# zz9tf/FIA-KDD-19

Hardware: AMD Instinct MI355X
Metric: influence queries/sec (whole node) + % HBM roofline, MF k=16 ML-1M-ex (higher is better)
Workload: dtype f64

## Files before the change

### fia-kdd-19_amd/csrc/common.h

```cpp
#pragma once

#include <hip/hip_runtime.h>
#include <hip/hip_ext.h>
#include <cstdint>
#include <cstdio>
#include <string>
#include <vector>

#include "fia.h"

namespace fia {

constexpr int kWave = 64;
constexpr int kScoreThreads = 256;
constexpr int kScoreRows = 4;
constexpr int kChunk = 64 * kScoreRows;
constexpr int kRunQB = 16;
constexpr int kRunChunk = 128;
constexpr int kNcfRunChunk = 64;
constexpr int kRunUserCost = 3;

struct ChunkDesc {
  int64_t list_base;
  int64_t out_base;
  int32_t q;
  int32_t pos0;
  int32_t len;
  int32_t side;
};
constexpr int kPrepThreads = 256;
constexpr int kSolveThreads = 64;
constexpr int kGramChunk = 256;
constexpr int kGsSub = 16;
constexpr int kGsSlice = 256;
constexpr int kGsTarget = 8;
constexpr uint32_t kGsNoRow = 0x7fffff00u;
constexpr int kGsRing = 8;
constexpr int kGsMaxSub = 48;
constexpr int kGsMaxSeg = 4;
constexpr int kMfmaQB = 16;
constexpr int kMfmaCPI = 4;
constexpr int kWgBlocks = 4;
constexpr int kQueryBlock = 8;
static_assert(kGsSlice < 512, "a Gram-stream segment's count rides in 9 bits of its descriptor (out >> 23)");

struct DevBuf {
  void* ptr = nullptr;
  size_t bytes = 0;
  hipError_t reserve(size_t want, hipStream_t s) {
    if (want <= bytes && ptr) return hipSuccess;
    hipStreamCaptureStatus cs = hipStreamCaptureStatusNone;
    if (hipStreamIsCapturing(s, &cs) == hipSuccess && cs != hipStreamCaptureStatusNone)
      return hipErrorStreamCaptureUnsupported;
    size_t cap = want < 256 ? 256 : want;
    if (ptr) {
      const size_t grown = bytes + bytes / 4;
      if (grown > cap) cap = grown;
      hipError_t e = hipFreeAsync(ptr, s);
      if (e != hipSuccess) return e;
      ptr = nullptr;
      bytes = 0;
    }
    hipError_t e = hipMallocAsync(&ptr, cap, s);
    if (e == hipSuccess) bytes = cap; else ptr = nullptr;
    return e;
  }
  void release(hipStream_t s) {
    if (ptr) (void)hipFreeAsync(ptr, s);
    ptr = nullptr;
    bytes = 0;
  }
  template <class T> T* as() const { return reinterpret_cast<T*>(ptr); }
};

struct Side {
  DevBuf ptr;
  DevBuf row;
  DevBuf other;
  DevBuf rating;
};

struct Index {
  int64_t N = 0, U = 0, I = 0;
  Side side[2];
  DevBuf order[2];
  DevBuf gitems[2], gcomb[2];
  int64_t n_gitems[2] = {0, 0}, n_gcomb[2] = {0, 0}, n_gslots[2] = {0, 0};
  DevBuf pkey;
  DevBuf pcnt;
  DevBuf psum;
  int64_t pcap = 0;
  std::vector<int64_t> hptr[2];
  std::vector<int32_t> hord[2];
  int64_t gchunk = 0;
  DevBuf gsdesc, gsids, gswave, gscomb[2];
  int64_t n_gsw = 0, n_gsdesc = 0, n_gscomb[2] = {0, 0}, n_gsslots[2] = {0, 0};
  uint64_t gs_version = ~0ull;
  int gs_k = 0;
  uint64_t version = 0;
  bool valid = false;
};

#define FIA_SMALL_SIZES(X) X(MF, 8) X(MF, 16) X(MF, 32) X(MF, 64) X(NCF, 8) X(NCF, 16) X(NCF, 32)
#define FIA_BIG_SIZES(X) X(MF, 128) X(MF, 256) X(NCF, 64) X(NCF, 128) X(NCF, 256)

#define FIA_SIZE_CASE(fam, kv)                \
  if (model == FIA_MODEL_##fam && k == kv) {  \
    f(fam<kv>{});                             \
    return true;                              \
  }
template <template <int> class MF, template <int> class NCF, class F>
bool for_small_size(int model, int k, F&& f) {
  FIA_SMALL_SIZES(FIA_SIZE_CASE)
  return false;
}
template <template <int> class MF, template <int> class NCF, class F>
bool for_big_size(int model, int k, F&& f) {
  FIA_BIG_SIZES(FIA_SIZE_CASE)
  return false;
}
#undef FIA_SIZE_CASE

template <class I, class T>
__device__ __forceinline__ I last_at_most(const T* __restrict__ off, I lo, I hi, T g) {
  while (lo < hi) {
    const I mid = (lo + hi + 1) >> 1;
    if (off[mid] <= g) lo = mid; else hi = mid - 1;
  }
  return lo;
}

constexpr unsigned long long kEmptyKey = ~0ull;

__host__ __device__ inline unsigned long long pair_hash(unsigned long long k) {
  k += 0x9e3779b97f4a7c15ull;
  k = (k ^ (k >> 30)) * 0xbf58476d1ce4e5b9ull;
  k = (k ^ (k >> 27)) * 0x94d049bb133111ebull;
  return k ^ (k >> 31);
}

struct PairTable {
  const unsigned long long* key;
  const int32_t* cnt;
  const double* sum;
  unsigned long long mask;
  __device__ inline void lookup(unsigned long long k, double& c, double& s) const {
    unsigned long long h = pair_hash(k) & mask;
    c = 0.0;
    s = 0.0;
    for (unsigned long long probe = 0; probe <= mask; ++probe) {
      unsigned long long kk = key[h];
      if (kk == k) { c = (double)cnt[h]; s = sum[h]; return; }
      if (kk == kEmptyKey) return;
      h = (h + 1) & mask;
    }
  }
  __device__ inline void probe_start(unsigned long long k, unsigned long long& h, unsigned long long& kk) const {
    h = pair_hash(k) & mask;
    kk = key[h];
  }
  __device__ inline void probe_finish(unsigned long long k, unsigned long long h, unsigned long long kk, double& c,
                                      double& s) const {
    c = 0.0;
    s = 0.0;
    for (unsigned long long probe = 0; probe <= mask; ++probe) {
      if (kk == k) { c = (double)cnt[h]; s = sum[h]; return; }
      if (kk == kEmptyKey) return;
      h = (h + 1) & mask;
      kk = key[h];
    }
  }
};

struct Params {
  int model = -1, k = 0;
  int64_t U = 0, I = 0;
  const float* t[10] = {};
  double wd = 0.0, damping = 0.0;
  bool valid = false;
};

struct PhaseEvents {
  std::vector<std::pair<hipEvent_t, hipEvent_t>> ev[FIA_NUM_PHASES];
  std::vector<hipEvent_t> pool;
};

struct RecHead {
  static constexpr int inv_n = 0;
  static constexpr int c_q = 1;
  static constexpr int x_v = 2;
  static constexpr int rhat = 3;
};

}

struct fia_ctx {
  int device = 0;
  std::string err;
  fia::Params p;
  fia::Index idx;
  fia::DevBuf gram[2];
  fia::DevBuf l1[2];
  fia::DevBuf gpart[2];
  bool prepared = false;
  fia::DevBuf rec;
  fia::DevBuf coff;
  fia::DevBuf cdesc;
  fia::DevBuf cand_pos;
  fia::DevBuf cand_val;
  fia::DevBuf qscan;
  fia::DevBuf flag;
  fia::DevBuf nch;
  fia::DevBuf coupled;
  fia::DevBuf gcnt;
  fia::DevBuf gstart;
  fia::DevBuf grank;
  fia::DevBuf gq;
  fia::DevBuf qbase;
  fia::DevBuf slices;
  fia::DevBuf wstart;
  fia::DevBuf gscan;
  fia::DevBuf witems;
  fia::DevBuf d1tab;
  fia::DevBuf tkeys, tvals, tagg, tslot, tword, tsort;
  fia::DevBuf rowrec, gxq;
  uint64_t rowrec_version = ~0ull;
  fia::DevBuf dwork, dslab, dpairs;
  fia::DevBuf self[2];
  uint64_t self_version = ~0ull;
  fia::DevBuf resid;
  fia::DevBuf gm[2];
  fia::DevBuf wfrag;
  fia::DevBuf slot[2];
  fia::DevBuf mark;
  bool subset = false;
  bool small_subset = false;
  fia::DevBuf bitems[2], bcomb[2];
  int64_t n_bitems[2] = {0, 0}, n_bcomb[2] = {0, 0}, n_bslots[2] = {0, 0}, n_bcache[2] = {0, 0};
  uint64_t bitems_version = ~0ull;
  int bitems_k = 0;
  fia::DevBuf qwork;
  fia::DevBuf xb;
  fia::DevBuf syslist;
  fia::DevBuf cpllist;
  fia::DevBuf lscr;
  int num_cus = 0;
  hipStream_t stream = nullptr;
  bool has_stream = false;
  hipStream_t aux = nullptr;
  hipEvent_t fork_ev = nullptr, prep_ev = nullptr;
  bool prep_pending = false;
  hipEvent_t l1_ev = nullptr;
  bool l1_pending = false;
  unsigned profiling = 0;
  fia::PhaseEvents events;
};

namespace fia {

struct ModelArgs {
  int64_t U, I;
  const int64_t* ptr[2];
  const float* t[10];
  const double* l1[2];
  double wd;
};
template <class Args>
void fill_model_args(const fia_ctx* c, Args& A) {
  A.U = c->p.U;
  A.I = c->p.I;
  for (int s = 0; s < 2; ++s) {
    A.ptr[s] = c->idx.side[s].ptr.as<int64_t>();
    A.l1[s] = c->l1[s].as<double>();
  }
  for (int j = 0; j < 10; ++j) A.t[j] = c->p.t[j];
  A.wd = c->p.wd;
}

inline PairTable pair_table(const Index& X) {
  return {X.pkey.as<unsigned long long>(), X.pcnt.as<int32_t>(), X.psum.as<double>(),
          (unsigned long long)(X.pcap - 1)};
}

template <class Args>
void fill_list_args(const fia_ctx* c, Args& A) {
  fill_model_args(c, A);
  for (int s = 0; s < 2; ++s) {
    A.row[s] = c->idx.side[s].row.as<int32_t>();
    A.other[s] = c->idx.side[s].other.as<int32_t>();
    A.rating[s] = c->idx.side[s].rating.as<float>();
    A.gram[s] = c->gram[s].as<double>();
  }
  A.damping = c->p.damping;
  A.pairs = pair_table(c->idx);
}

hipError_t build_index(fia_ctx* c, int64_t N, int64_t U, int64_t I, const int32_t* user,
                       const int32_t* item, const float* rating, hipStream_t s, std::string& why);
hipError_t count_related(fia_ctx* c, int64_t Q, const int32_t* qu, const int32_t* qi,
                         int64_t* offsets, hipStream_t s);
hipError_t write_related(fia_ctx* c, int64_t Q, const int32_t* qu, const int32_t* qi,
                         const int64_t* offsets, int32_t* rel, hipStream_t s);
hipError_t build_chunks(fia_ctx* c, int64_t Q, const int32_t* qu, const int32_t* qi, const int64_t* offsets,
                        int64_t max_chunks, bool offsets_only, hipStream_t s, int32_t* zero_word = nullptr,
                        bool runs = false, int slice_cost = 0, int run_chunk = kRunChunk);
hipError_t build_gram_lists(fia_ctx* c, int64_t chunk, hipStream_t s);
hipError_t build_gram_stream(fia_ctx* c, int k, hipStream_t s);
hipError_t build_groups(fia_ctx* c, int64_t Q, const int32_t* qu, const int32_t* qi, const int64_t* offsets,
                        int64_t max_items, int qb, hipStream_t s, int cpi = 1);

hipError_t prepare_model(fia_ctx* c, hipStream_t s, bool& unsupported);
hipStream_t prepare_stream(fia_ctx* c, hipStream_t s);
hipError_t prepare_record(fia_ctx* c, hipStream_t ps, hipStream_t s);
hipError_t join_prepare(fia_ctx* c, hipStream_t s);
hipError_t join_l1(fia_ctx* c, hipStream_t s);
hipError_t prepare_model_for(fia_ctx* c, int64_t Q, const int32_t* qu, const int32_t* qi, hipStream_t s, hipStream_t ps,
                             bool& unsupported, bool mark_only);
hipError_t mark_entities(fia_ctx* c, int64_t Q, const int32_t* qu, const int32_t* qi, hipStream_t s);
hipError_t check_cover_small(fia_ctx* c, int64_t Q, const int32_t* qu, const int32_t* qi, int32_t* flag,
                             hipStream_t s);
hipError_t query_model(fia_ctx* c, int64_t Q, const int32_t* qu, const int32_t* qi, const int64_t* offsets,
                       int64_t max_chunks, int32_t* rel_idx, double* influence, double* x_out, int K,
                       int64_t* topk_pos, int64_t* topk_idx, double* topk_val, hipStream_t s,
                       bool& unsupported,
                       const double* x_in = nullptr);
int model_num_params(int model, int k);
bool model_supported(int model, int k);

bool big_supported(int model, int k);
hipError_t ensure_self(fia_ctx* c, hipStream_t s);
int live_contexts(int device);
hipError_t prepare_big(fia_ctx* c, int64_t Q, const int32_t* qu, const int32_t* qi, hipStream_t s);
hipError_t check_cover(fia_ctx* c, int64_t Q, const int32_t* qu, const int32_t* qi, int32_t* flag, hipStream_t s);
hipError_t query_big(fia_ctx* c, int64_t Q, const int32_t* qu, const int32_t* qi, const int64_t* offsets,
                     int64_t max_chunks, int32_t* rel_idx, double* influence, double* x_out, int K,
                     int64_t* topk_pos, int64_t* topk_idx, double* topk_val, hipStream_t s,
                     const double* x_in = nullptr);
struct PhaseSpan {
  hipEvent_t a = nullptr, b = nullptr;
};
struct QueryArgs;
struct GramStreamArgs {
  const int2* desc;
  const uint32_t* ids;
  const int32_t* wave;
  int64_t n_waves;
  const float* emb_other[2];
  uint32_t bytes_other[2];
  double* gram[2];
  double* part[2];
  const uint8_t* mark;
  int64_t moff[2];
};
hipError_t launch_gram_mf_stream(int k, const GramStreamArgs& G, hipStream_t s);
hipError_t launch_score_mf_runs(int k, int64_t grid, hipStream_t s, const QueryArgs& A, int64_t Q,
                                const ChunkDesc* cdesc, const int64_t* qbase, const int32_t* slices,
                                const double* rec, int32_t* rel_idx, double* influence, int K, int32_t* cand_pos,
                                double* cand_val, PhaseSpan ps);
hipError_t launch_score_ncf_runs(int k, int64_t grid, hipStream_t s, const QueryArgs& A, int64_t Q,
                                 const ChunkDesc* cdesc, const int64_t* qbase, const int32_t* slices,
                                 const double* rec, int32_t* rel_idx, double* influence, int K, int32_t* cand_pos,
                                 double* cand_val, PhaseSpan ps);
hipError_t launch_score_mf_mfma(int k, bool full, int64_t grid, hipStream_t s, PhaseSpan ps, const QueryArgs& A,
                                int64_t nE, const int64_t* wstart, const int32_t* witems, const int64_t* gstart,
                                const int32_t* gq, const int64_t* qbase, const double* rec, int32_t* rel_idx,
                                double* influence, int K, int32_t* cand_pos, double* cand_val);
hipError_t launch_topk_merge(fia_ctx* c, int64_t Q, const int32_t* qu, const int32_t* qi, int K, int spc,
                             int64_t* topk_pos, int64_t* topk_idx, double* topk_val, hipStream_t s,
                             int64_t max_chunks);

hipError_t score_candidates(fia_ctx* c, int64_t Q, const int32_t* qu, const int32_t* qi, const double* x,
                            const int64_t* cand_offsets, int64_t total_cand, const int32_t* cand_user,
                            const int32_t* cand_item, const float* cand_rating, double* influence, int K,
                            int64_t* topk_pos, double* topk_val, hipStream_t s);

hipError_t total_influence(fia_ctx* c, int64_t Q, const int32_t* qu, const int32_t* qi, const double* x,
                           double* total, int32_t* count, int K, int64_t* topk_idx, double* topk_val,
                           hipStream_t s);

hipError_t big_systems(fia_ctx* c, int64_t Q, const int32_t* qu, const int32_t* qi, bool solve, bool sides,
                       hipStream_t s);

hipError_t ensure_rowrec(fia_ctx* c, hipStream_t s);
hipError_t group_influence_big(fia_ctx* c, int64_t Q, const int32_t* qu, const int32_t* qi,
                               const int64_t* grp_offsets, int64_t num_groups, const int64_t* mem_offsets,
                               int64_t total_members, const int32_t* mem_row, double* group, double* first_order,
                               double* dtheta, hipStream_t s);
hipError_t self_influence_big(fia_ctx* c, int64_t n, const int32_t* rows, double* first_order, double* newton,
                              double* error, hipStream_t s);
bool group_supported(int model, int k);
hipError_t group_influence(fia_ctx* c, int64_t Q, const int32_t* qu, const int32_t* qi, const int64_t* grp_offsets,
                           int64_t num_groups, const int64_t* mem_offsets, int64_t total_members,
                           const int32_t* mem_row, double* group, double* first_order, double* dtheta,
                           hipStream_t s);

hipError_t self_influence(fia_ctx* c, int64_t n, const int32_t* rows, double* first_order, double* newton,
                          double* error, int K, int64_t* topk_pos, int64_t* topk_idx, double* topk_val,
                          hipStream_t s);

bool newton_supported(int model, int k);
hipError_t query_newton(fia_ctx* c, int64_t Q, const int32_t* qu, const int32_t* qi, const int64_t* offsets,
                        int64_t total_rel, int32_t* rel_idx, double* newton, int K, int64_t* topk_pos,
                        int64_t* topk_idx, double* topk_val, hipStream_t s);

void phase_begin(fia_ctx* c, int phase, hipStream_t s);
void phase_end(fia_ctx* c, int phase, hipStream_t s);
PhaseSpan phase_span(fia_ctx* c, int phase);
void phase_drop(fia_ctx* c, int phase, const PhaseSpan& ps);

}

#define FIA_HIP_TRY(expr)                       \
  do {                                          \
    hipError_t _e = (expr);                     \
    if (_e != hipSuccess) return _e;            \
  } while (0)
```

### fia-kdd-19_amd/csrc/gram_mf.hip

```cpp
#include "kern.h"

namespace fia {
namespace {

constexpr int kRsrcWord3 = 0x00020000;

template <class M, bool MARK>
__global__ __launch_bounds__(64) void k_gram_mf_stream(GramStreamArgs G) {
  static_assert(!M::ncf && M::K <= 16, "MF k <= 16");
  constexpr int K = M::K, Ds = M::Ds, GS = Ds * (Ds + 1) / 2, GSP = (GS + 1) & ~1;
  static_assert(kGsRing == 8 && kGsMaxSub % kGsRing == 0 && kGsMaxSub + kGsRing <= 64, "ring of 8");
  __shared__ __attribute__((aligned(16))) double stage[kGsMaxSeg][GSP];
  __shared__ uint4 sids[kGsMaxSub * 4];
  const int64_t w = blockIdx.x;
  if (w >= G.n_waves) return;
  const int d0 = G.wave[w], nd = G.wave[w + 1] - d0;
  const int lane = threadIdx.x;
  const int col = lane & 15, grp = lane >> 4;
  const int2 dv = lane < nd ? G.desc[d0 + lane] : int2{1 << 7, 0};
  bool sk = (dv.x >> 7) & 1;
  if constexpr (MARK) sk = sk || !G.mark[((dv.x >> 6) & 1 ? G.moff[1] : G.moff[0]) + (dv.x >> 8)];
  const uint64_t skipm = __ballot(sk), lastm = __ballot((dv.x >> 5) & 1), sidem = __ballot((dv.x >> 6) & 1);
  if (MARK && skipm == ~0ull) return;
  {
    const uint4* __restrict__ src = reinterpret_cast<const uint4*>(G.ids) + (int64_t)d0 * 4;
    uint4 tmp[kGsMaxSub * 4 / 64];
#pragma unroll
    for (int r = 0; r < kGsMaxSub * 4 / 64; ++r) {
      const int i = r * 64 + lane;
      tmp[r] = src[i < nd * 4 ? i : 0];
    }
#pragma unroll
    for (int r = 0; r < kGsMaxSub * 4 / 64; ++r) sids[r * 64 + lane] = tmp[r];
    wave_lds_sync();
  }
  const __amdgpu_buffer_rsrc_t rs0 =
      __builtin_amdgcn_make_buffer_rsrc(const_cast<float*>(G.emb_other[0]), 0, G.bytes_other[0], kRsrcWord3);
  const __amdgpu_buffer_rsrc_t rs1 =
      __builtin_amdgcn_make_buffer_rsrc(const_cast<float*>(G.emb_other[1]), 0, G.bytes_other[1], kRsrcWord3);
  const uint32_t cb = col < K ? (uint32_t)col * 4u : 0x80000000u;
  auto rows = [&](int t, float (&v)[4]) {
    const __amdgpu_buffer_rsrc_t rs = (sidem >> t) & 1 ? rs1 : rs0;
    const uint32_t sb = t >= nd || (MARK && ((skipm >> t) & 1)) ? 0x80000000u : 0u;
    const uint4 o4 = sids[(t < nd ? t : 0) * 4 + grp];
    const uint32_t oq[4] = {o4.x, o4.y, o4.z, o4.w};
#pragma unroll
    for (int q = 0; q < 4; ++q) {
      const uint32_t off = (oq[q] + cb) | sb;
      v[q] = __uint_as_float(__builtin_amdgcn_raw_buffer_load_b32(rs, (int)off, 0, 0));
    }
  };
  d4_t acc0 = {0.0, 0.0, 0.0, 0.0}, acc1 = {0.0, 0.0, 0.0, 0.0};
  double sum = 0.0;
  int nseg = 0;
  auto step = [&](int t, const float (&vin)[4]) {
    if ((skipm >> t) & 1) return;
    float v[4] = {vin[0], vin[1], vin[2], vin[3]};
    asm volatile("" : "+v"(v[0]), "+v"(v[1]), "+v"(v[2]), "+v"(v[3]));
    double g[4];
#pragma unroll
    for (int q = 0; q < 4; ++q) g[q] = (double)v[q];
    acc0 = __builtin_amdgcn_mfma_f64_16x16x4f64(g[0], g[0], acc0, 0, 0, 0);
    acc1 = __builtin_amdgcn_mfma_f64_16x16x4f64(g[1], g[1], acc1, 0, 0, 0);
    acc0 = __builtin_amdgcn_mfma_f64_16x16x4f64(g[2], g[2], acc0, 0, 0, 0);
    acc1 = __builtin_amdgcn_mfma_f64_16x16x4f64(g[3], g[3], acc1, 0, 0, 0);
    sum += (g[0] + g[1]) + (g[2] + g[3]);
    if (!((lastm >> t) & 1)) return;
    const uint32_t out = (uint32_t)__builtin_amdgcn_readlane(dv.y, t);
    double* __restrict__ st = stage[nseg];
    double cs = sum;
    cs += __shfl_xor(cs, 16);
    cs += __shfl_xor(cs, 32);
#pragma unroll
    for (int rr = 0; rr < 4; ++rr) {
      const int row = grp + 4 * rr;
      if (row < K && col <= row) st[tri(row, col)] = acc0[rr] + acc1[rr];
    }
    if (grp == 0 && col < K) st[tri(K, col)] = cs;
    if (lane == 0) st[tri(K, K)] = (double)(out >> 23);
    if (GSP > GS && lane == 1) st[GSP - 1] = 0.0;
    ++nseg;
    acc0 = acc1 = d4_t{0.0, 0.0, 0.0, 0.0};
    sum = 0.0;
  };
  constexpr int AH = kGsRing - 2;
  float r[kGsRing][4];
#pragma unroll
  for (int j = 0; j < AH; ++j) rows(j, r[j]);
  for (int t = 0; t < nd; t += kGsRing) {
#pragma unroll
    for (int j = 0; j < kGsRing; ++j) {
      rows(t + j + AH, r[(j + AH) % kGsRing]);
      step(t + j, r[j]);
    }
  }
  wave_lds_sync();
  uint64_t ends = lastm & ~skipm;
  for (int k = 0; k < nseg; ++k) {
    const int t = (int)__builtin_ctzll(ends);
    ends &= ends - 1;
    const int meta = __builtin_amdgcn_readlane(dv.x, t);
    const uint32_t out = (uint32_t)__builtin_amdgcn_readlane(dv.y, t);
    const int sd = (meta >> 6) & 1, e = meta >> 8, slot = (int)(out & 0x7fffffu) - 1;
    double* __restrict__ o = slot < 0 ? G.gram[sd] + (int64_t)e * GSP : G.part[sd] + (int64_t)slot * GSP;
#pragma unroll
    for (int b = 0; b < GSP; b += 128)
      if (b + 2 * lane < GSP)
        *reinterpret_cast<double2*>(o + b + 2 * lane) = *reinterpret_cast<const double2*>(&stage[k][b + 2 * lane]);
  }
}

}

hipError_t launch_gram_mf_stream(int k, const GramStreamArgs& G, hipStream_t s) {
  if (G.n_waves <= 0) return hipSuccess;
  const dim3 grid((unsigned)G.n_waves), blk(64);
  if (k == 16) {
    if (G.mark) hipLaunchKernelGGL((k_gram_mf_stream<MFm<16>, true>), grid, blk, 0, s, G);
    else hipLaunchKernelGGL((k_gram_mf_stream<MFm<16>, false>), grid, blk, 0, s, G);
  } else if (k == 8) {
    if (G.mark) hipLaunchKernelGGL((k_gram_mf_stream<MFm<8>, true>), grid, blk, 0, s, G);
    else hipLaunchKernelGGL((k_gram_mf_stream<MFm<8>, false>), grid, blk, 0, s, G);
  } else {
    return hipErrorInvalidValue;
  }
  return hipGetLastError();
}

}
```

### fia-kdd-19_amd/csrc/index.hip

```cpp
#include <algorithm>
#include <cstdlib>
#include <cstring>
#include <rocprim/device/device_radix_sort.hpp>
#include <rocprim/iterator/counting_iterator.hpp>

#include "common.h"
#include "scan.h"

namespace fia {
namespace {

__global__ void k_check_ids(const int32_t* __restrict__ user, const int32_t* __restrict__ item, int64_t N,
                            int64_t U, int64_t I, int32_t* __restrict__ flag) {
  int64_t j = (int64_t)blockIdx.x * blockDim.x + threadIdx.x;
  int64_t stride = (int64_t)gridDim.x * blockDim.x;
  int bad = 0;
  for (; j < N; j += stride) {
    int32_t u = user[j], i = item[j];
    bad |= (u < 0 || u >= U || i < 0 || i >= I);
  }
  if (__any(bad) && (threadIdx.x & 63) == 0) atomicOr(flag, 1);
}

__global__ void k_gather_side(const int32_t* __restrict__ rows, const int32_t* __restrict__ other_src,
                              const float* __restrict__ rating_src, int64_t N, int32_t* __restrict__ other,
                              float* __restrict__ rating) {
  int64_t j = (int64_t)blockIdx.x * blockDim.x + threadIdx.x;
  int64_t stride = (int64_t)gridDim.x * blockDim.x;
  for (; j < N; j += stride) {
    int32_t r = rows[j];
    other[j] = other_src[r];
    rating[j] = rating_src[r];
  }
}

__global__ void k_pair_insert(const int32_t* __restrict__ user, const int32_t* __restrict__ item,
                              const float* __restrict__ rating, int64_t N, int64_t I, unsigned long long* key,
                              int32_t* cnt, double* sum, unsigned long long mask) {
  int64_t j = (int64_t)blockIdx.x * blockDim.x + threadIdx.x;
  int64_t stride = (int64_t)gridDim.x * blockDim.x;
  for (; j < N; j += stride) {
    const unsigned long long k = (unsigned long long)user[j] * (unsigned long long)I + (unsigned long long)item[j];
    unsigned long long h = pair_hash(k) & mask;
    for (unsigned long long probe = 0; probe <= mask; ++probe) {
      unsigned long long prev = atomicCAS(&key[h], kEmptyKey, k);
      if (prev == kEmptyKey || prev == k) {
        atomicAdd(&cnt[h], 1);
        atomicAdd(&sum[h], (double)rating[j]);
        break;
      }
      h = (h + 1) & mask;
    }
  }
}

__global__ void k_list_ptr(const int32_t* __restrict__ keys, int64_t N, int64_t n_entity, int64_t* __restrict__ ptr) {
  int64_t e = (int64_t)blockIdx.x * blockDim.x + threadIdx.x;
  if (e > n_entity) return;
  int64_t lo = 0, hi = N;
  while (lo < hi) {
    int64_t mid = (lo + hi) >> 1;
    if (keys[mid] < e) lo = mid + 1; else hi = mid;
  }
  ptr[e] = lo;
}

__device__ inline void query_sides(const int32_t* qu, const int32_t* qi, int64_t q, const int64_t* uptr,
                                   const int64_t* iptr, int64_t U, int64_t I, int64_t& ub, int64_t& du, int64_t& ib,
                                   int64_t& di) {
  const int32_t u = qu[q], i = qi[q];
  ub = du = ib = di = 0;
  if (u >= 0 && u < U && i >= 0 && i < I) {
    ub = uptr[u];
    du = uptr[u + 1] - ub;
    ib = iptr[i];
    di = iptr[i + 1] - ib;
  }
}

template <int MODE>
__global__ __launch_bounds__(kScanThreads) void k_query_scan(
    const int32_t* __restrict__ qu, const int32_t* __restrict__ qi, int64_t Q, const int64_t* __restrict__ uptr,
    const int64_t* __restrict__ iptr, int64_t U, int64_t I, int64_t* __restrict__ out,
    unsigned long long* __restrict__ tstate, unsigned int* __restrict__ tctr, int32_t* __restrict__ flag,
    const int64_t* __restrict__ offsets, ChunkDesc* __restrict__ cdesc, int32_t* __restrict__ zero_word,
    int64_t* __restrict__ qbase, int runs, int clen, int lsh, int32_t* __restrict__ slices) {
  query_scan_body<MODE>(qu, qi, Q, uptr, iptr, U, I, out, tstate, tctr, flag, offsets, cdesc, zero_word, qbase, runs,
                        clen, lsh, slices);
}

__global__ void k_group_count(const int32_t* __restrict__ qu, const int32_t* __restrict__ qi, int64_t Q,
                              const int64_t* __restrict__ uptr, const int64_t* __restrict__ iptr, int64_t U, int64_t I,
                              const int64_t* __restrict__ offsets, const int64_t* __restrict__ coff,
                              unsigned long long* __restrict__ gcnt, int32_t* __restrict__ grank,
                              int64_t* __restrict__ qbase) {
  const int64_t q = (int64_t)blockIdx.x * blockDim.x + threadIdx.x;
  if (q >= Q) return;
  int64_t ub, du, ib, di;
  query_sides(qu, qi, q, uptr, iptr, U, I, ub, du, ib, di);
  const int32_t u = qu[q], i = qi[q];
  const bool ok = (u >= 0 && u < U && i >= 0 && i < I) && (du + di > 0);
  grank[2 * q] = ok ? (int32_t)atomicAdd(&gcnt[u], 1ull) : -1;
  grank[2 * q + 1] = ok ? (int32_t)atomicAdd(&gcnt[U + i], 1ull) : -1;
  qbase[4 * q + 0] = offsets[q];
  qbase[4 * q + 1] = offsets[q] + du;
  qbase[4 * q + 2] = coff[q];
  qbase[4 * q + 3] = coff[q] + (du + kChunk - 1) / kChunk;
}

__global__ void k_group_fill(const int32_t* __restrict__ qu, const int32_t* __restrict__ qi, int64_t Q, int64_t U,
                             const int64_t* __restrict__ gstart, const int32_t* __restrict__ grank,
                             int32_t* __restrict__ gq) {
  const int64_t t = (int64_t)blockIdx.x * blockDim.x + threadIdx.x;
  if (t < Q && grank[2 * t] >= 0) {
    const int32_t u = qu[t], i = qi[t];
    gq[gstart[u] + grank[2 * t]] = (int32_t)t;
    gq[gstart[U + i] + grank[2 * t + 1]] = (int32_t)t;
  }
}

__global__ __launch_bounds__(kScanThreads) void k_group_scan(
    unsigned long long* __restrict__ gcnt, const int64_t* __restrict__ uptr, const int64_t* __restrict__ iptr,
    int64_t U, int64_t I, int qb, int cpi, int64_t* __restrict__ gstart, int64_t* __restrict__ wstart,
    unsigned long long* __restrict__ tstate, unsigned int* __restrict__ tctr) {
  __shared__ int s_tile;
  __shared__ int64_t s_wa[kScanThreads / 64], s_wb[kScanThreads / 64];
  __shared__ int64_t s_pa, s_pb;
  const int64_t nE = U + I;
  const unsigned ntiles = (unsigned)((nE + 1 + kScanTile - 1) / kScanTile);
  if (threadIdx.x == 0) s_tile = (int)atomicAdd(&tctr[0], 1u);
  __syncthreads();
  const int64_t tile = s_tile;
  const int lane = threadIdx.x & 63, wave = threadIdx.x >> 6;
  const int64_t t = tile * kScanTile + threadIdx.x;
  int64_t a = 0, b = 0;
  if (t < nE) {
    a = (int64_t)gcnt[t];
    if (a > 0) gcnt[t] = 0;
    if (a > 0) {
      const int64_t deg = t < U ? uptr[t + 1] - uptr[t] : iptr[t - U + 1] - iptr[t - U];
      b = ((deg + kChunk * cpi - 1) / (kChunk * cpi)) * ((a + qb - 1) / qb);
    }
  }
  int64_t ia = a, ib = b;
#pragma unroll
  for (int off = 1; off < 64; off <<= 1) {
    const int64_t ya = __shfl_up(ia, off), yb = __shfl_up(ib, off);
    if (lane >= off) { ia += ya; ib += yb; }
  }
  if (lane == 63) { s_wa[wave] = ia; s_wb[wave] = ib; }
  __syncthreads();
  int64_t ba = 0, bb = 0, agg_a = 0, agg_b = 0;
#pragma unroll
  for (int w = 0; w < kScanThreads / 64; ++w) {
    if (w < wave) { ba += s_wa[w]; bb += s_wb[w]; }
    agg_a += s_wa[w];
    agg_b += s_wb[w];
  }
  if (wave == 0) {
    const int64_t ea = scan_lookback(tstate, tile, agg_a);
    const int64_t eb = scan_lookback(tstate + ntiles, tile, agg_b);
    if (lane == 0) { s_pa = ea; s_pb = eb; }
  }
  __syncthreads();
  if (t <= nE) {
    gstart[t] = s_pa + ba + ia - a;
    wstart[t] = s_pb + bb + ib - b;
  }
  __syncthreads();
  if (threadIdx.x == 0) {
    asm volatile("s_waitcnt vmcnt(0)" ::: "memory");
    const unsigned done = atomicAdd(&tctr[1], 1u);
    if (done == ntiles - 1) {
      for (unsigned w = 0; w < 2 * ntiles; ++w)
        __hip_atomic_store(&tstate[w], 0ull, __ATOMIC_RELAXED, __HIP_MEMORY_SCOPE_AGENT);
      __hip_atomic_store(&tctr[0], 0u, __ATOMIC_RELAXED, __HIP_MEMORY_SCOPE_AGENT);
      __hip_atomic_store(&tctr[1], 0u, __ATOMIC_RELAXED, __HIP_MEMORY_SCOPE_AGENT);
    }
  }
}

__global__ void k_item_fill(const int64_t* __restrict__ wstart, const int64_t* __restrict__ gstart,
                            int64_t nE, int32_t* __restrict__ witems, int qb) {
  const int64_t total = wstart[nE];
  for (int64_t w = (int64_t)blockIdx.x * blockDim.x + threadIdx.x; w < total;
       w += (int64_t)gridDim.x * blockDim.x) {
    const int64_t lo = last_at_most(wstart, (int64_t)0, nE - 1, w);
    const int64_t b = wstart[lo];
    const int64_t nqb = (gstart[lo + 1] - gstart[lo] + qb - 1) / qb;
    witems[3 * w] = (int32_t)lo;
    witems[3 * w + 1] = (int32_t)((w - b) / nqb);
    witems[3 * w + 2] = (int32_t)((w - b) % nqb);
  }
}

__global__ void k_write_related(const int32_t* __restrict__ qu, const int32_t* __restrict__ qi,
                                const int64_t* __restrict__ offsets, const int64_t* __restrict__ uptr,
                                const int32_t* __restrict__ urow, const int64_t* __restrict__ iptr,
                                const int32_t* __restrict__ irow, int64_t U, int64_t I, int32_t* __restrict__ rel) {
  int64_t q = blockIdx.x;
  int32_t u = qu[q], i = qi[q];
  if (u < 0 || u >= U || i < 0 || i >= I) return;
  int64_t base = offsets[q];
  int64_t ub = uptr[u], du = uptr[u + 1] - ub;
  int64_t ib = iptr[i], di = iptr[i + 1] - ib;
  for (int64_t p = threadIdx.x; p < du; p += blockDim.x) rel[base + p] = urow[ub + p];
  for (int64_t p = threadIdx.x; p < di; p += blockDim.x) rel[base + du + p] = irow[ib + p];
}

}

namespace {

inline unsigned bits_for(int64_t n) {
  unsigned b = 1;
  while (b < 31 && ((int64_t)1 << b) < n) ++b;
  return b;
}

inline int grid_for(int64_t n, int threads, int cap = 8192) {
  int64_t g = (n + threads - 1) / threads;
  if (g < 1) g = 1;
  if (g > cap) g = cap;
  return (int)g;
}

}

hipError_t build_gram_lists(fia_ctx* c, int64_t chunk, hipStream_t s) {
  Index& X = c->idx;
  for (int sd = 0; sd < 2; ++sd) {
    const std::vector<int64_t>& hptr = X.hptr[sd];
    std::vector<int32_t> items, comb;
    int32_t slots = 0;
    for (int32_t e : X.hord[sd]) {
      const int64_t len = hptr[(size_t)e + 1] - hptr[(size_t)e];
      const int64_t nit = len == 0 ? 1 : (len + chunk - 1) / chunk;
      if (nit > 1) comb.insert(comb.end(), {e, slots, (int32_t)nit, 0});
      for (int64_t t = 0; t < nit; ++t) {
        const int64_t st = t * chunk;
        const int64_t ln = std::min<int64_t>(chunk, len - st);
        items.insert(items.end(), {e, (int32_t)st, (int32_t)(ln < 0 ? 0 : ln), nit > 1 ? slots++ : -1});
      }
    }
    X.n_gitems[sd] = (int64_t)items.size() / 4;
    X.n_gcomb[sd] = (int64_t)comb.size() / 4;
    X.n_gslots[sd] = slots;
    if (!items.empty()) {
      FIA_HIP_TRY(X.gitems[sd].reserve(sizeof(int32_t) * items.size(), s));
      FIA_HIP_TRY(hipMemcpyAsync(X.gitems[sd].ptr, items.data(), sizeof(int32_t) * items.size(), hipMemcpyHostToDevice, s));
    }
    if (!comb.empty()) {
      FIA_HIP_TRY(X.gcomb[sd].reserve(sizeof(int32_t) * comb.size(), s));
      FIA_HIP_TRY(hipMemcpyAsync(X.gcomb[sd].ptr, comb.data(), sizeof(int32_t) * comb.size(), hipMemcpyHostToDevice, s));
    }
    FIA_HIP_TRY(hipStreamSynchronize(s));
  }
  X.gchunk = chunk;
  return hipSuccess;
}

__global__ void k_gs_ids(int64_t nd, const int2* __restrict__ desc, const int32_t* __restrict__ pos,
                         const int32_t* __restrict__ other0, const int32_t* __restrict__ other1, int k,
                         uint32_t* __restrict__ ids) {
  for (int64_t t = (int64_t)blockIdx.x * blockDim.x + threadIdx.x; t < nd * kGsSub;
       t += (int64_t)gridDim.x * blockDim.x) {
    const int64_t d = t / kGsSub;
    const int r = 4 * (int)(t & 3) + (int)((t >> 2) & 3);
    const int meta = desc[d].x;
    const int valid = meta & 31, side = (meta >> 6) & 1;
    ids[t] = r < valid ? (uint32_t)(side ? other1 : other0)[pos[d] + r] * (uint32_t)(k * 4) : kGsNoRow;
  }
}

hipError_t build_gram_stream(fia_ctx* c, int k, hipStream_t s) {
  Index& X = c->idx;
  if (X.gs_version == X.version && X.gs_k == k && X.gswave.ptr) return hipSuccess;
  struct Seg {
    int64_t len;
    int side;
    int32_t e, start, slot;
  };
  std::vector<Seg> segs;
  std::vector<int32_t> comb[2];
  for (int sd = 0; sd < 2; ++sd) {
    const std::vector<int64_t>& hptr = X.hptr[sd];
    int32_t slots = 0;
    for (int32_t e : X.hord[sd]) {
      const int64_t len = hptr[(size_t)e + 1] - hptr[(size_t)e];
      if (len <= kGsSlice) {
        segs.push_back({len, sd, e, 0, -1});
        continue;
      }
      const int64_t nit = (len + kGsSlice - 1) / kGsSlice;
      comb[sd].insert(comb[sd].end(), {e, slots, (int32_t)nit, 0});
      for (int64_t t = 0; t < nit; ++t)
        segs.push_back({std::min<int64_t>(kGsSlice, len - t * kGsSlice), sd, e, (int32_t)(t * kGsSlice), slots++});
    }
    X.n_gsslots[sd] = slots;
  }
  std::stable_sort(segs.begin(), segs.end(), [](const Seg& a, const Seg& b) { return a.len > b.len; });
  std::vector<int2> desc;
  std::vector<int32_t> pos, wave{0};
  int cur = 0, nseg = 0;
  auto close_wave = [&]() {
    while (cur % kGsRing) {
      desc.push_back(int2{1 << 7, -1});
      pos.push_back(0);
      ++cur;
    }
    wave.push_back((int32_t)desc.size());
    cur = 0;
    nseg = 0;
  };
  for (const Seg& g : segs) {
    const int nsb = g.len == 0 ? 1 : (int)((g.len + kGsSub - 1) / kGsSub);
    if (cur > 0 && cur + nsb > kGsMaxSub - kGsRing) close_wave();
    for (int t = 0; t < nsb; ++t) {
      const int valid = (int)std::min<int64_t>(kGsSub, g.len - (int64_t)t * kGsSub);
      const bool last = t == nsb - 1;
      const int meta = (valid < 0 ? 0 : valid) | (last ? 1 << 5 : 0) | (g.side << 6) | (g.e << 8);
      const uint32_t out = last ? ((uint32_t)g.len << 23) | (uint32_t)(g.slot + 1) : 0u;
      desc.push_back(int2{meta, (int)out});
      pos.push_back((int32_t)(X.hptr[g.side][(size_t)g.e] + g.start + (int64_t)t * kGsSub));
    }
    cur += nsb;
    if (cur >= kGsTarget || ++nseg >= kGsMaxSeg) close_wave();
  }
  if (cur > 0) close_wave();
  const int64_t nd = (int64_t)desc.size();
  X.n_gsdesc = nd;
  X.n_gsw = (int64_t)wave.size() - 1;
  FIA_HIP_TRY(X.gsdesc.reserve(sizeof(int2) * (size_t)(nd + 2), s));
  FIA_HIP_TRY(X.gsids.reserve(sizeof(int32_t) * (size_t)((nd + 2) * kGsSub), s));
  FIA_HIP_TRY(X.gswave.reserve(sizeof(int32_t) * wave.size(), s));
  DevBuf dpos;
  FIA_HIP_TRY(dpos.reserve(sizeof(int32_t) * (size_t)(nd + 1), s));
  if (nd > 0) {
    FIA_HIP_TRY(hipMemcpyAsync(X.gsdesc.ptr, desc.data(), sizeof(int2) * (size_t)nd, hipMemcpyHostToDevice, s));
    FIA_HIP_TRY(hipMemcpyAsync(dpos.ptr, pos.data(), sizeof(int32_t) * (size_t)nd, hipMemcpyHostToDevice, s));
    hipLaunchKernelGGL(k_gs_ids, dim3(grid_for(nd * kGsSub, 256)), dim3(256), 0, s, nd, X.gsdesc.as<int2>(),
                       dpos.as<int32_t>(), X.side[0].other.as<int32_t>(), X.side[1].other.as<int32_t>(), k,
                       X.gsids.as<uint32_t>());
    FIA_HIP_TRY(hipGetLastError());
  }
  FIA_HIP_TRY(hipMemsetAsync(X.gsdesc.as<int2>() + nd, 0, sizeof(int2) * 2, s));
  FIA_HIP_TRY(hipMemcpyAsync(X.gswave.ptr, wave.data(), sizeof(int32_t) * wave.size(), hipMemcpyHostToDevice, s));
  for (int sd = 0; sd < 2; ++sd) {
    X.n_gscomb[sd] = (int64_t)comb[sd].size() / 4;
    if (!comb[sd].empty()) {
      FIA_HIP_TRY(X.gscomb[sd].reserve(sizeof(int32_t) * comb[sd].size(), s));
      FIA_HIP_TRY(hipMemcpyAsync(X.gscomb[sd].ptr, comb[sd].data(), sizeof(int32_t) * comb[sd].size(),
                                 hipMemcpyHostToDevice, s));
    }
  }
  dpos.release(s);
  FIA_HIP_TRY(hipStreamSynchronize(s));
  X.gs_version = X.version;
  X.gs_k = k;
  return hipSuccess;
}

hipError_t build_index(fia_ctx* c, int64_t N, int64_t U, int64_t I, const int32_t* user, const int32_t* item,
                       const float* rating, hipStream_t s, std::string& why) {
  Index& X = c->idx;
  X.valid = false;
  FIA_HIP_TRY(c->flag.reserve(64, s));
  FIA_HIP_TRY(hipMemsetAsync(c->flag.ptr, 0, 64, s));
  if (N > 0) {
    hipLaunchKernelGGL(k_check_ids, dim3(grid_for(N, 256)), dim3(256), 0, s, user, item, N, U, I,
                       c->flag.as<int32_t>());
    FIA_HIP_TRY(hipGetLastError());
  }
  int32_t hflag = 0;
  FIA_HIP_TRY(hipMemcpyAsync(&hflag, c->flag.ptr, sizeof(int32_t), hipMemcpyDeviceToHost, s));
  FIA_HIP_TRY(hipStreamSynchronize(s));
  if (hflag) {
    why = "training ids out of range [0, num_users) x [0, num_items)";
    return hipErrorInvalidValue;
  }
  DevBuf keys_sorted, tmp;
  FIA_HIP_TRY(keys_sorted.reserve(sizeof(int32_t) * (size_t)(N > 0 ? N : 1), s));
  const int32_t* key_src[2] = {user, item};
  const int32_t* other_src[2] = {item, user};
  int64_t n_ent[2] = {U, I};
  for (int sd = 0; sd < 2; ++sd) {
    Side& S = X.side[sd];
    size_t nb = sizeof(int32_t) * (size_t)(N > 0 ? N : 1);
    FIA_HIP_TRY(S.row.reserve(nb, s));
    FIA_HIP_TRY(S.other.reserve(nb, s));
    FIA_HIP_TRY(S.rating.reserve(sizeof(float) * (size_t)(N > 0 ? N : 1), s));
    FIA_HIP_TRY(S.ptr.reserve(sizeof(int64_t) * (size_t)(n_ent[sd] + 1), s));
    if (N > 0) {
      unsigned eb = bits_for(n_ent[sd]);
      rocprim::counting_iterator<int32_t> iota(0);
      size_t tb = 0;
      FIA_HIP_TRY(rocprim::radix_sort_pairs(nullptr, tb, key_src[sd], keys_sorted.as<int32_t>(), iota,
                                            S.row.as<int32_t>(), (size_t)N, 0u, eb, s));
      FIA_HIP_TRY(tmp.reserve(tb + 16, s));
      tb = tmp.bytes;
      FIA_HIP_TRY(rocprim::radix_sort_pairs(tmp.ptr, tb, key_src[sd], keys_sorted.as<int32_t>(), iota,
                                            S.row.as<int32_t>(), (size_t)N, 0u, eb, s));
      hipLaunchKernelGGL(k_gather_side, dim3(grid_for(N, 256)), dim3(256), 0, s, S.row.as<int32_t>(),
                         other_src[sd], rating, N, S.other.as<int32_t>(), S.rating.as<float>());
      FIA_HIP_TRY(hipGetLastError());
    }
    hipLaunchKernelGGL(k_list_ptr, dim3((unsigned)((n_ent[sd] + 1 + 255) / 256)), dim3(256), 0, s,
                       keys_sorted.as<int32_t>(), N, n_ent[sd], S.ptr.as<int64_t>());
    FIA_HIP_TRY(hipGetLastError());
    FIA_HIP_TRY(hipStreamSynchronize(s));
    std::vector<int64_t> hptr((size_t)n_ent[sd] + 1);
    FIA_HIP_TRY(hipMemcpyAsync(hptr.data(), S.ptr.ptr, sizeof(int64_t) * hptr.size(), hipMemcpyDeviceToHost, s));
    FIA_HIP_TRY(hipStreamSynchronize(s));
    std::vector<int32_t> ord((size_t)n_ent[sd]);
    for (int64_t e = 0; e < n_ent[sd]; ++e) ord[(size_t)e] = (int32_t)e;
    std::stable_sort(ord.begin(), ord.end(), [&](int32_t a, int32_t b) {
      return hptr[(size_t)a + 1] - hptr[(size_t)a] > hptr[(size_t)b + 1] - hptr[(size_t)b];
    });
    X.hptr[sd] = hptr;
    FIA_HIP_TRY(X.order[sd].reserve(sizeof(int32_t) * ord.size(), s));
    FIA_HIP_TRY(hipMemcpyAsync(X.order[sd].ptr, ord.data(), sizeof(int32_t) * ord.size(), hipMemcpyHostToDevice, s));
    FIA_HIP_TRY(hipStreamSynchronize(s));
    X.hord[sd] = ord;
  }
  FIA_HIP_TRY(build_gram_lists(c, kGramChunk, s));
  keys_sorted.release(s);
  tmp.release(s);
  int64_t cap = 1024;
  while (cap < 2 * N) cap <<= 1;
  FIA_HIP_TRY(X.pkey.reserve(sizeof(unsigned long long) * (size_t)cap, s));
  FIA_HIP_TRY(X.pcnt.reserve(sizeof(int32_t) * (size_t)cap, s));
  FIA_HIP_TRY(X.psum.reserve(sizeof(double) * (size_t)cap, s));
  FIA_HIP_TRY(hipMemsetAsync(X.pkey.ptr, 0xff, sizeof(unsigned long long) * (size_t)cap, s));
  FIA_HIP_TRY(hipMemsetAsync(X.pcnt.ptr, 0, sizeof(int32_t) * (size_t)cap, s));
  FIA_HIP_TRY(hipMemsetAsync(X.psum.ptr, 0, sizeof(double) * (size_t)cap, s));
  if (N > 0) {
    hipLaunchKernelGGL(k_pair_insert, dim3(grid_for(N, 256)), dim3(256), 0, s, user, item, rating, N, I,
                       X.pkey.as<unsigned long long>(), X.pcnt.as<int32_t>(), X.psum.as<double>(),
                       (unsigned long long)(cap - 1));
    FIA_HIP_TRY(hipGetLastError());
  }
  FIA_HIP_TRY(hipStreamSynchronize(s));
  X.pcap = cap;
  ++X.version;
  X.N = N;
  X.U = U;
  X.I = I;
  X.valid = true;
  return hipSuccess;
}

static hipError_t scan_state(fia_ctx* c, int64_t Q, hipStream_t s) {
  const int64_t ntiles = (Q + 1 + kScanTile - 1) / kScanTile;
  const size_t need = sizeof(unsigned long long) * (size_t)(2 * ntiles) + 16;
  if (c->qscan.bytes >= need && c->qscan.ptr) return hipSuccess;
  FIA_HIP_TRY(c->qscan.reserve(need < 4096 ? 4096 : need, s));
  FIA_HIP_TRY(hipMemsetAsync(c->qscan.ptr, 0, c->qscan.bytes, s));
  return hipSuccess;
}

static hipError_t query_scan_args(fia_ctx* c, int64_t Q, const int32_t* qu, const int32_t* qi, int64_t* out,
                                  const int64_t* offsets, ChunkDesc* cdesc, int32_t* zero_word, hipStream_t s,
                                  int64_t* qbase, int runs, int clen, int lsh, int32_t* slices, ScanArgs& S) {
  FIA_HIP_TRY(scan_state(c, Q, s));
  FIA_HIP_TRY(c->flag.reserve(64, s));
  unsigned int* ctr = reinterpret_cast<unsigned int*>(c->qscan.as<char>() + c->qscan.bytes - 16);
  S = ScanArgs{qu, qi, Q, c->idx.side[0].ptr.as<int64_t>(), c->idx.side[1].ptr.as<int64_t>(), c->idx.U, c->idx.I, out,
               c->qscan.as<unsigned long long>(), ctr, c->flag.as<int32_t>(), offsets, cdesc, zero_word, qbase, runs,
               clen, lsh, slices};
  return hipSuccess;
}

template <int MODE>
static hipError_t launch_query_scan(const ScanArgs& S, hipStream_t s, hipEvent_t ev_a, hipEvent_t ev_b) {
  hipExtLaunchKernelGGL(k_query_scan<MODE>, dim3((unsigned)scan_tiles(S.Q)), dim3(kScanThreads), 0, s, ev_a, ev_b, 0,
                        S.qu, S.qi, S.Q, S.uptr, S.iptr, S.U, S.I, S.out, S.tstate, S.tctr, S.flag, S.offsets, S.cdesc,
                        S.zero_word, S.qbase, S.runs, S.clen, S.lsh, S.slices);
  return hipGetLastError();
}

hipError_t count_related(fia_ctx* c, int64_t Q, const int32_t* qu, const int32_t* qi, int64_t* offsets,
                         hipStream_t s) {
  ScanArgs S;
  FIA_HIP_TRY(query_scan_args(c, Q, qu, qi, offsets, nullptr, nullptr, nullptr, s, nullptr, 0, kChunk, 0, nullptr, S));
  return launch_query_scan<0>(S, s, nullptr, nullptr);
}

hipError_t write_related(fia_ctx* c, int64_t Q, const int32_t* qu, const int32_t* qi, const int64_t* offsets,
                         int32_t* rel, hipStream_t s) {
  if (Q == 0) return hipSuccess;
  hipLaunchKernelGGL(k_write_related, dim3((unsigned)Q), dim3(256), 0, s, qu, qi, offsets,
                     c->idx.side[0].ptr.as<int64_t>(), c->idx.side[0].row.as<int32_t>(),
                     c->idx.side[1].ptr.as<int64_t>(), c->idx.side[1].row.as<int32_t>(), c->idx.U, c->idx.I, rel);
  return hipGetLastError();
}


hipError_t chunk_scan_args(fia_ctx* c, int64_t Q, const int32_t* qu, const int32_t* qi, const int64_t* offsets,
                           int64_t max_chunks, bool offsets_only, hipStream_t s, int32_t* zero_word, bool runs,
                           int slice_cost, int run_chunk, ScanArgs& S) {
  FIA_HIP_TRY(c->coff.reserve(sizeof(int64_t) * (size_t)(Q + 1), s));
  const bool rq = runs && !offsets_only;
  if (!offsets_only) FIA_HIP_TRY(c->cdesc.reserve(sizeof(ChunkDesc) * (size_t)(max_chunks + 1), s));
  int lsh = 0;
  while ((1 << lsh) < slice_cost && lsh < 30) ++lsh;
  const int lam = 1 << lsh;
  if (rq) {
    FIA_HIP_TRY(c->qbase.reserve(sizeof(int64_t) * (size_t)(4 * Q + 2), s));
    FIA_HIP_TRY(c->slices.reserve(sizeof(int32_t) * (size_t)((max_chunks + 1) * (kRunQB + 2) / lam + 2), s));
  }
  return query_scan_args(c, Q, qu, qi, c->coff.as<int64_t>(), offsets,
                         offsets_only ? nullptr : c->cdesc.as<ChunkDesc>(), zero_word, s,
                         rq ? c->qbase.as<int64_t>() : nullptr, rq ? kRunQB : 0, rq ? run_chunk : kChunk, lsh,
                         rq ? c->slices.as<int32_t>() : nullptr, S);
}

hipError_t launch_chunk_scan(const ScanArgs& S, hipStream_t s, hipEvent_t ev_a, hipEvent_t ev_b) {
  return launch_query_scan<1>(S, s, ev_a, ev_b);
}

hipError_t build_chunks(fia_ctx* c, int64_t Q, const int32_t* qu, const int32_t* qi, const int64_t* offsets,
                        int64_t max_chunks, bool offsets_only, hipStream_t s, int32_t* zero_word, bool runs,
                        int slice_cost, int run_chunk) {
  ScanArgs S;
  FIA_HIP_TRY(chunk_scan_args(c, Q, qu, qi, offsets, max_chunks, offsets_only, s, zero_word, runs, slice_cost,
                              run_chunk, S));
  return launch_chunk_scan(S, s);
}

hipError_t build_groups(fia_ctx* c, int64_t Q, const int32_t* qu, const int32_t* qi, const int64_t* offsets,
                        int64_t max_items, int qb, hipStream_t s, int cpi) {
  const int64_t U = c->idx.U, I = c->idx.I, nE = U + I;
  const int64_t ntiles = (nE + 1 + kScanTile - 1) / kScanTile;
  if (c->gcnt.bytes < sizeof(int64_t) * (size_t)(nE + 1) || !c->gcnt.ptr) {
    FIA_HIP_TRY(c->gcnt.reserve(sizeof(int64_t) * (size_t)(nE + 1), s));
    FIA_HIP_TRY(hipMemsetAsync(c->gcnt.ptr, 0, c->gcnt.bytes, s));
  }
  FIA_HIP_TRY(c->gstart.reserve(sizeof(int64_t) * (size_t)(nE + 1), s));
  FIA_HIP_TRY(c->wstart.reserve(sizeof(int64_t) * (size_t)(nE + 1), s));
  FIA_HIP_TRY(c->grank.reserve(sizeof(int32_t) * (size_t)(2 * Q + 1), s));
  FIA_HIP_TRY(c->gq.reserve(sizeof(int32_t) * (size_t)(2 * Q + 1), s));
  FIA_HIP_TRY(c->qbase.reserve(sizeof(int64_t) * (size_t)(4 * Q + 1), s));
  FIA_HIP_TRY(c->witems.reserve(sizeof(int32_t) * (size_t)(3 * max_items + 3), s));
  const size_t need = sizeof(unsigned long long) * (size_t)(2 * ntiles) + 16;
  if (c->gscan.bytes < need || !c->gscan.ptr) {
    FIA_HIP_TRY(c->gscan.reserve(need, s));
    FIA_HIP_TRY(hipMemsetAsync(c->gscan.ptr, 0, c->gscan.bytes, s));
  }
  const int64_t* uptr = c->idx.side[0].ptr.as<int64_t>();
  const int64_t* iptr = c->idx.side[1].ptr.as<int64_t>();
  if (Q > 0) {
    hipLaunchKernelGGL(k_group_count, dim3((unsigned)((Q + 255) / 256)), dim3(256), 0, s, qu, qi, Q, uptr, iptr, U, I,
                       offsets, c->coff.as<int64_t>(), c->gcnt.as<unsigned long long>(), c->grank.as<int32_t>(),
                       c->qbase.as<int64_t>());
    FIA_HIP_TRY(hipGetLastError());
  }
  unsigned int* ctr = reinterpret_cast<unsigned int*>(c->gscan.as<char>() + c->gscan.bytes - 16);
  hipLaunchKernelGGL(k_group_scan, dim3((unsigned)ntiles), dim3(kScanThreads), 0, s, c->gcnt.as<unsigned long long>(),
                     uptr, iptr, U, I, qb, cpi, c->gstart.as<int64_t>(), c->wstart.as<int64_t>(),
                     c->gscan.as<unsigned long long>(), ctr);
  FIA_HIP_TRY(hipGetLastError());
  if (Q > 0) {
    hipLaunchKernelGGL(k_group_fill, dim3((unsigned)((Q + 255) / 256)), dim3(256), 0, s, qu, qi, Q, U,
                       c->gstart.as<int64_t>(), c->grank.as<int32_t>(), c->gq.as<int32_t>());
    FIA_HIP_TRY(hipGetLastError());
  }
  hipLaunchKernelGGL(k_item_fill, dim3(grid_for(max_items, 256, 16384)), dim3(256), 0, s, c->wstart.as<int64_t>(),
                     c->gstart.as<int64_t>(), nE, c->witems.as<int32_t>(), qb);
  return hipGetLastError();
}

}
```

Measured before the change: 132.2 million.

## Split mid-length Gram segments across a 4-wave workgroup team and reduce in LDS

The Gram-stream kernel now runs four waves per workgroup. Entities whose history spans a few slices no longer write per-slice partials to global memory for a later combine step. Instead their slices are spread over the waves of one workgroup, and the first wave sums the staged partial Grams from shared memory and writes the final Gram directly. The host-side wave builder packs these teams and the remaining segment ranges into groups of four, padding with empty ranges. This trades fewer global partial writes and combine work for a block-wide barrier, more LDS per block, and possible idle padded waves.

```diff
diff --git a/fia-kdd-19_amd/csrc/common.h b/fia-kdd-19_amd/csrc/common.h
--- a/fia-kdd-19_amd/csrc/common.h
+++ b/fia-kdd-19_amd/csrc/common.h
@@ -38,11 +38,19 @@
 constexpr int kGsRing = 8;
 constexpr int kGsMaxSub = 48;
 constexpr int kGsMaxSeg = 4;
+constexpr int kGsWaves = 4;
+constexpr int kGsTeamPer = kGsMaxSub / (kGsSlice / kGsSub);
+constexpr int kGsTeamSlices = kGsWaves * kGsTeamPer;
+constexpr int kGsTeamMinPer = 1;
+constexpr uint32_t kGsTeamBit = 1u << 22;
 constexpr int kMfmaQB = 16;
 constexpr int kMfmaCPI = 4;
 constexpr int kWgBlocks = 4;
 constexpr int kQueryBlock = 8;
 static_assert(kGsSlice < 512, "a Gram-stream segment's count rides in 9 bits of its descriptor (out >> 23)");
+static_assert(kGsSlice % kGsSub == 0 && kGsTeamPer >= 1 && kGsTeamPer <= kGsMaxSeg && kGsTeamPer < 8 &&
+                  kGsTeamSlices < 32,
+              "a team wave stages its slices from segment 0; slice and count ride in 5 bits each, per in 3");
 
 struct DevBuf {
   void* ptr = nullptr;
diff --git a/fia-kdd-19_amd/csrc/gram_mf.hip b/fia-kdd-19_amd/csrc/gram_mf.hip
--- a/fia-kdd-19_amd/csrc/gram_mf.hip
+++ b/fia-kdd-19_amd/csrc/gram_mf.hip
@@ -6,32 +6,32 @@
 constexpr int kRsrcWord3 = 0x00020000;
 
 template <class M, bool MARK>
-__global__ __launch_bounds__(64) void k_gram_mf_stream(GramStreamArgs G) {
+__global__ __launch_bounds__(64 * kGsWaves) void k_gram_mf_stream(GramStreamArgs G) {
   static_assert(!M::ncf && M::K <= 16, "MF k <= 16");
   constexpr int K = M::K, Ds = M::Ds, GS = Ds * (Ds + 1) / 2, GSP = (GS + 1) & ~1;
   static_assert(kGsRing == 8 && kGsMaxSub % kGsRing == 0 && kGsMaxSub + kGsRing <= 64, "ring of 8");
-  __shared__ __attribute__((aligned(16))) double stage[kGsMaxSeg][GSP];
-  __shared__ uint4 sids[kGsMaxSub * 4];
-  const int64_t w = blockIdx.x;
-  if (w >= G.n_waves) return;
-  const int d0 = G.wave[w], nd = G.wave[w + 1] - d0;
-  const int lane = threadIdx.x;
+  __shared__ __attribute__((aligned(16))) double stage_all[kGsWaves][kGsMaxSeg][GSP];
+  __shared__ uint4 sids_all[kGsWaves][kGsMaxSub * 4];
+  const int wid = __builtin_amdgcn_readfirstlane((int)threadIdx.x >> 6);
+  double (*const stage)[GSP] = stage_all[wid];
+  uint4* const sids = sids_all[wid];
+  const int64_t w = (int64_t)blockIdx.x * kGsWaves + wid;
+  const int d0 = G.wave[w], nd0 = G.wave[w + 1] - d0;
+  const int lane = threadIdx.x & 63;
   const int col = lane & 15, grp = lane >> 4;
-  const int2 dv = lane < nd ? G.desc[d0 + lane] : int2{1 << 7, 0};
+  const int2 dv = lane < nd0 ? G.desc[d0 + lane] : int2{1 << 7, 0};
   bool sk = (dv.x >> 7) & 1;
   if constexpr (MARK) sk = sk || !G.mark[((dv.x >> 6) & 1 ? G.moff[1] : G.moff[0]) + (dv.x >> 8)];
   const uint64_t skipm = __ballot(sk), lastm = __ballot((dv.x >> 5) & 1), sidem = __ballot((dv.x >> 6) & 1);
-  if (MARK && skipm == ~0ull) return;
-  {
+  const int nd = skipm == ~0ull ? 0 : nd0;
+  if (nd > 0) {
     const uint4* __restrict__ src = reinterpret_cast<const uint4*>(G.ids) + (int64_t)d0 * 4;
-    uint4 tmp[kGsMaxSub * 4 / 64];
-#pragma unroll
-    for (int r = 0; r < kGsMaxSub * 4 / 64; ++r) {
-      const int i = r * 64 + lane;
-      tmp[r] = src[i < nd * 4 ? i : 0];
-    }
-#pragma unroll
-    for (int r = 0; r < kGsMaxSub * 4 / 64; ++r) sids[r * 64 + lane] = tmp[r];
+    static_assert(kGsMaxSub * 4 == 3 * 64, "three 16-B words per lane");
+    const int n4 = nd * 4;
+    const uint4 t0 = src[lane < n4 ? lane : 0], t1 = src[64 + lane < n4 ? 64 + lane : 0], t2 = src[128 + lane < n4 ? 128 + lane : 0];
+    sids[lane] = t0;
+    sids[64 + lane] = t1;
+    sids[128 + lane] = t2;
     wave_lds_sync();
   }
   const __amdgpu_buffer_rsrc_t rs0 =
@@ -85,8 +85,10 @@
   };
   constexpr int AH = kGsRing - 2;
   float r[kGsRing][4];
+  if (nd > 0) {
 #pragma unroll
-  for (int j = 0; j < AH; ++j) rows(j, r[j]);
+    for (int j = 0; j < AH; ++j) rows(j, r[j]);
+  }
   for (int t = 0; t < nd; t += kGsRing) {
 #pragma unroll
     for (int j = 0; j < kGsRing; ++j) {
@@ -94,15 +96,35 @@
       step(t + j, r[j]);
     }
   }
-  wave_lds_sync();
+  __syncthreads();
   uint64_t ends = lastm & ~skipm;
   for (int k = 0; k < nseg; ++k) {
     const int t = (int)__builtin_ctzll(ends);
     ends &= ends - 1;
     const int meta = __builtin_amdgcn_readlane(dv.x, t);
     const uint32_t out = (uint32_t)__builtin_amdgcn_readlane(dv.y, t);
-    const int sd = (meta >> 6) & 1, e = meta >> 8, slot = (int)(out & 0x7fffffu) - 1;
-    double* __restrict__ o = slot < 0 ? G.gram[sd] + (int64_t)e * GSP : G.part[sd] + (int64_t)slot * GSP;
+    const int sd = (meta >> 6) & 1, e = meta >> 8;
+    double* const gram_e = (sd ? G.gram[1] : G.gram[0]) + (int64_t)e * GSP;
+    if (out & kGsTeamBit) {
+      if ((out >> 8) & 31) continue;
+      const int ns = (int)(out >> 3) & 31, per = (int)out & 7;
+      double* __restrict__ o = gram_e;
+#pragma unroll
+      for (int b = 0; b < GSP; b += 128)
+        if (b + 2 * lane < GSP) {
+          double2 a = {0.0, 0.0};
+          for (int j = 0, ww = wid, kk = 0; j < ns; ++j) {
+            const double2 v = *reinterpret_cast<const double2*>(&stage_all[ww][kk][b + 2 * lane]);
+            a.x += v.x;
+            a.y += v.y;
+            if (++kk == per) kk = 0, ++ww;
+          }
+          *reinterpret_cast<double2*>(o + b + 2 * lane) = a;
+        }
+      continue;
+    }
+    const int slot = (int)(out & 0x7fffffu) - 1;
+    double* __restrict__ o = slot < 0 ? gram_e : (sd ? G.part[1] : G.part[0]) + (int64_t)slot * GSP;
 #pragma unroll
     for (int b = 0; b < GSP; b += 128)
       if (b + 2 * lane < GSP)
@@ -114,7 +136,8 @@
 
 hipError_t launch_gram_mf_stream(int k, const GramStreamArgs& G, hipStream_t s) {
   if (G.n_waves <= 0) return hipSuccess;
-  const dim3 grid((unsigned)G.n_waves), blk(64);
+  if (G.n_waves % kGsWaves) return hipErrorInvalidValue;
+  const dim3 grid((unsigned)(G.n_waves / kGsWaves)), blk(64 * kGsWaves);
   if (k == 16) {
     if (G.mark) hipLaunchKernelGGL((k_gram_mf_stream<MFm<16>, true>), grid, blk, 0, s, G);
     else hipLaunchKernelGGL((k_gram_mf_stream<MFm<16>, false>), grid, blk, 0, s, G);
diff --git a/fia-kdd-19_amd/csrc/index.hip b/fia-kdd-19_amd/csrc/index.hip
--- a/fia-kdd-19_amd/csrc/index.hip
+++ b/fia-kdd-19_amd/csrc/index.hip
@@ -281,7 +281,17 @@
     int side;
     int32_t e, start, slot;
   };
+  struct Team {
+    int64_t len;
+    int side;
+    int32_t e, nit;
+  };
+  struct Range {
+    std::vector<int2> d;
+    std::vector<int32_t> p;
+  };
   std::vector<Seg> segs;
+  std::vector<Team> teams;
   std::vector<int32_t> comb[2];
   for (int sd = 0; sd < 2; ++sd) {
     const std::vector<int64_t>& hptr = X.hptr[sd];
@@ -293,41 +303,85 @@
         continue;
       }
       const int64_t nit = (len + kGsSlice - 1) / kGsSlice;
+      if (nit <= kGsTeamSlices) {
+        teams.push_back({len, sd, e, (int32_t)nit});
+        continue;
+      }
       comb[sd].insert(comb[sd].end(), {e, slots, (int32_t)nit, 0});
       for (int64_t t = 0; t < nit; ++t)
         segs.push_back({std::min<int64_t>(kGsSlice, len - t * kGsSlice), sd, e, (int32_t)(t * kGsSlice), slots++});
     }
+    if ((uint32_t)slots >= kGsTeamBit) return hipErrorInvalidValue;
     X.n_gsslots[sd] = slots;
   }
+  std::stable_sort(teams.begin(), teams.end(), [](const Team& a, const Team& b) { return a.len > b.len; });
   std::stable_sort(segs.begin(), segs.end(), [](const Seg& a, const Seg& b) { return a.len > b.len; });
-  std::vector<int2> desc;
-  std::vector<int32_t> pos, wave{0};
-  int cur = 0, nseg = 0;
-  auto close_wave = [&]() {
-    while (cur % kGsRing) {
-      desc.push_back(int2{1 << 7, -1});
-      pos.push_back(0);
-      ++cur;
-    }
-    wave.push_back((int32_t)desc.size());
-    cur = 0;
-    nseg = 0;
-  };
-  for (const Seg& g : segs) {
+  auto emit = [&](Range& r, const Seg& g, uint32_t out_low) {
     const int nsb = g.len == 0 ? 1 : (int)((g.len + kGsSub - 1) / kGsSub);
-    if (cur > 0 && cur + nsb > kGsMaxSub - kGsRing) close_wave();
     for (int t = 0; t < nsb; ++t) {
       const int valid = (int)std::min<int64_t>(kGsSub, g.len - (int64_t)t * kGsSub);
       const bool last = t == nsb - 1;
       const int meta = (valid < 0 ? 0 : valid) | (last ? 1 << 5 : 0) | (g.side << 6) | (g.e << 8);
-      const uint32_t out = last ? ((uint32_t)g.len << 23) | (uint32_t)(g.slot + 1) : 0u;
-      desc.push_back(int2{meta, (int)out});
-      pos.push_back((int32_t)(X.hptr[g.side][(size_t)g.e] + g.start + (int64_t)t * kGsSub));
-    }
-    cur += nsb;
-    if (cur >= kGsTarget || ++nseg >= kGsMaxSeg) close_wave();
-  }
-  if (cur > 0) close_wave();
+      const uint32_t out = last ? ((uint32_t)g.len << 23) | out_low : 0u;
+      r.d.push_back(int2{meta, (int)out});
+      r.p.push_back((int32_t)(X.hptr[g.side][(size_t)g.e] + g.start + (int64_t)t * kGsSub));
+    }
+    return nsb;
+  };
+  auto close = [&](Range& r) {
+    while (r.d.size() % kGsRing) {
+      r.d.push_back(int2{1 << 7, -1});
+      r.p.push_back(0);
+    }
+  };
+  std::vector<std::vector<Range>> wgs;
+  for (const Team& tm : teams) {
+    const int per = std::max(kGsTeamMinPer, (tm.nit + kGsWaves - 1) / kGsWaves), nw = (tm.nit + per - 1) / per;
+    if (wgs.empty() || (int)wgs.back().size() + nw > kGsWaves) wgs.emplace_back();
+    std::vector<Range>& wg = wgs.back();
+    for (int32_t j = 0; j < tm.nit; ++j) {
+      if (j % per == 0) wg.emplace_back();
+      const Seg g{std::min<int64_t>(kGsSlice, tm.len - (int64_t)j * kGsSlice), tm.side, tm.e, j * kGsSlice, -1};
+      emit(wg.back(), g, kGsTeamBit | (uint32_t)j << 8 | (uint32_t)tm.nit << 3 | (uint32_t)per);
+      if (j % per == per - 1 || j == tm.nit - 1) close(wg.back());
+    }
+  }
+  size_t fill = 0;
+  auto place = [&](Range&& r) {
+    close(r);
+    while (fill < wgs.size() && (int)wgs[fill].size() >= kGsWaves) ++fill;
+    if (fill == wgs.size()) wgs.emplace_back();
+    wgs[fill].push_back(std::move(r));
+  };
+  {
+    Range r;
+    int cur = 0, nseg = 0;
+    for (const Seg& g : segs) {
+      const int nsb = g.len == 0 ? 1 : (int)((g.len + kGsSub - 1) / kGsSub);
+      if (cur > 0 && cur + nsb > kGsMaxSub - kGsRing) {
+        place(std::move(r));
+        r = Range{};
+        cur = nseg = 0;
+      }
+      cur += emit(r, g, (uint32_t)(g.slot + 1));
+      if (cur >= kGsTarget || ++nseg >= kGsMaxSeg) {
+        place(std::move(r));
+        r = Range{};
+        cur = nseg = 0;
+      }
+    }
+    if (cur > 0) place(std::move(r));
+  }
+  std::vector<int2> desc;
+  std::vector<int32_t> pos, wave{0};
+  for (std::vector<Range>& wg : wgs) {
+    wg.resize(kGsWaves);
+    for (const Range& r : wg) {
+      desc.insert(desc.end(), r.d.begin(), r.d.end());
+      pos.insert(pos.end(), r.p.begin(), r.p.end());
+      wave.push_back((int32_t)desc.size());
+    }
+  }
   const int64_t nd = (int64_t)desc.size();
   X.n_gsdesc = nd;
   X.n_gsw = (int64_t)wave.size() - 1;
```

Measured after the change: 134.5 million, median of 6. 1.02x the previous value.
